# vovach777/llcomp

Measured on AMD Instinct MI355X. Metric: encode+decode MPix/s on 4K RGB8, bit-exact, higher is better.
Workload: dtype int32

## Files before the change

### llcomp_amd/csrc/dec_rows_asm.hpp

```cpp
#pragma once
#include <cstdint>

namespace llcomp_mi {

#define LD_E0L "v32"
#define LD_E0H "v33"
#define LD_E0 "v[32:33]"
#define LD_E5L "v34"
#define LD_E5H "v35"
#define LD_E5 "v[34:35]"
#define LD_E6L "v36"
#define LD_E6H "v37"
#define LD_E6 "v[36:37]"
#define LD_E7L "v38"
#define LD_E7H "v39"
#define LD_E7 "v[38:39]"
#define LD_E1L "v40"
#define LD_E1H "v41"
#define LD_E1 "v[40:41]"
#define LD_E2L "v42"
#define LD_E2H "v43"
#define LD_E2 "v[42:43]"
#define LD_E3L "v44"
#define LD_E3H "v45"
#define LD_E3 "v[44:45]"
#define LD_E4L "v48"
#define LD_E4H "v49"
#define LD_E4 "v[48:49]"
#define LD_PROD "v50"
#define LD_R1 "v51"
#define LD_DIFF "v52"
#define LD_OFF "v52"
#define LD_EX "v32"
#define LD_W "v33"
#define LD_RUN "v40"
#define LD_NX "v41"
#define LD_T "v42"
#define LD_SX "s[56:57]"
#define LD_SA "s[58:59]"
#define LD_SW "s[60:61]"
#define LD_SP "s[62:63]"
#define LD_S5 "s[64:65]"
#define LD_SB "s[64:65]"
#define LD_SU "s[66:67]"
#define LD_SD "s[68:69]"
#define LD_S1L "s[68:69]"
#define LD_SM "s[70:71]"
#define LD_S1 "s70"
#define LD_S2 "s71"

#define LD_SPLIT(EL)                                                                                                       \
    "v_mul_u32_u24_sdwa " LD_PROD ", " EL ", %[range] dst_sel:DWORD dst_unused:UNUSED_PAD src0_sel:BYTE_1 src1_sel:DWORD\n\t" \
    "v_lshrrev_b32_e32 " LD_R1 ", 8, " LD_PROD "\n\t"                                                                      \
    "v_sub_u32_e32 %[range], %[range], " LD_R1 "\n\t"
#define LD_SPLIT_IN(EL)                                                                                                       \
    "v_mul_u32_u24_sdwa " LD_PROD ", " EL ", %[range_in] dst_sel:DWORD dst_unused:UNUSED_PAD src0_sel:BYTE_1 src1_sel:DWORD\n\t" \
    "v_lshrrev_b32_e32 " LD_R1 ", 8, " LD_PROD "\n\t"                                                                      \
    "v_sub_u32_e32 %[range], %[range_in], " LD_R1 "\n\t"
#define LD_SPLIT_TO(EL, RD, WR)                                                                                       \
    "v_mul_u32_u24_sdwa " LD_PROD ", " EL ", " RD " dst_sel:DWORD dst_unused:UNUSED_PAD src0_sel:BYTE_1 src1_sel:DWORD\n\t" \
    "v_lshrrev_b32_e32 " WR ", 8, " LD_PROD "\n\t"                                                                     \
    "v_sub_u32_e32 " RD ", " RD ", " WR "\n\t"
#define LD_TAKE "v_lshlrev_b64 " LD_PAIR ", 8, " LD_PAIR "\n"
#define LD_REFILL(N)                                         \
    "v_cmp_gt_u32_e32 vcc, %[c100], %[range]\n\t"            \
    "s_and_saveexec_b64 " LD_SW ", vcc\n\t"                  \
    "s_cbranch_execz .Lrf" N "_%=\n\t"                       \
    "v_lshlrev_b32_e32 %[range], 8, %[range]\n\t"            \
    LD_TAKE                                                  \
    ".Lrf" N "_%=:\n\t"                                      \
    "s_mov_b64 exec, " LD_SW "\n\t"
#define LD_REFILL_R1(WR, N)                                       \
    "v_cmp_gt_u32_e32 vcc, %[c100], " WR "\n\t"                   \
    "s_and_saveexec_b64 " LD_SW ", vcc\n\t"                       \
    "s_cbranch_execz .Lrf" N "_%=\n\t"                            \
    "v_and_b32_e32 " WR ", 0xffffff00, " LD_PROD "\n\t"           \
    LD_TAKE                                                       \
    ".Lrf" N "_%=:\n\t"                                           \
    "s_mov_b64 exec, " LD_SW "\n\t"
#define LD_UNARY(EL, EH, OFS, N, SAVE, RD, WR)                              \
    LD_SPLIT_TO(EL, RD, WR)                                                 \
    "v_sub_co_u32_e32 " LD_LOW ", vcc, " LD_LOW ", " RD "\n\t"              \
    "ds_write_b16_d16_hi %[bank], " EL " offset:" OFS "\n\t"                \
    "s_andn2_b64 exec, exec, vcc\n\t"                                       \
    SAVE                                                                    \
    "s_cbranch_execz .Lx_done_%=\n\t"                                       \
    "ds_write_b16_d16_hi %[bank], " EH " offset:" OFS "\n\t"                \
    "v_add_u32_e32 " LD_EX ", 1, " LD_EX "\n\t"                             \
    LD_REFILL_R1(WR, N)
#define LD_FETCH_REST                                         \
    "v_lshrrev_b32_e32 " LD_E1L ", 16, %[w0]\n\t"             \
    "v_and_b32_e32 " LD_E2L ", 0xffff, %[w1]\n\t"             \
    "v_lshrrev_b32_e32 " LD_E3L ", 16, %[w1]\n\t"             \
    "v_and_b32_e32 " LD_E4L ", 0xffff, %[w2]\n\t"             \
    "ds_read_b64 " LD_E1 ", " LD_E1L "\n\t"                   \
    "ds_read_b64 " LD_E2 ", " LD_E2L "\n\t"                   \
    "ds_read_b64 " LD_E3 ", " LD_E3L "\n\t"                   \
    "ds_read_b64 " LD_E4 ", " LD_E4L "\n\t"                   \
    "v_lshrrev_b32_e32 " LD_E5L ", 16, %[w2]\n\t"             \
    "v_and_b32_e32 " LD_E6L ", 0xffff, %[w3]\n\t"             \
    "v_lshrrev_b32_e32 " LD_E7L ", 16, %[w3]\n\t"             \
    "ds_read_b64 " LD_E5 ", " LD_E5L "\n\t"                   \
    "ds_read_b64 " LD_E6 ", " LD_E6L "\n\t"                   \
    "ds_read_b64 " LD_E7 ", " LD_E7L "\n\t"

#define LD_HEAD_COPY "v_perm_b32 " LD_CPY ", %[winl_in], %[winl_in], %[sel]\n\t"
#define LD_SEL 0x0001020Du
#define LD_TAIL_BITS "v_ffbl_b32_e32 " LD_DIFF ", " LD_CPY "\n\t"
#define LD_URUN                                                      \
    ".Lu_%=:\n\t"                                                    \
    "s_waitcnt lgkmcnt(0)\n\t"                                       \
    LD_SPLIT_TO(LD_E4L, LD_R1, "%[range]")                           \
    "v_sub_co_u32_e32 " LD_LOW ", vcc, " LD_LOW ", " LD_R1 "\n\t"    \
    "s_and_b64 " LD_SP ", exec, vcc\n\t"                             \
    "s_andn2_b64 exec, exec, vcc\n\t"                                \
    "s_or_b64 " LD_SB ", " LD_SB ", " LD_SP "\n\t"                   \
    "s_cbranch_execz .Lu_done_%=\n\t"                                \
    "v_lshrrev_b32_e32 " LD_OFF ", 16, " LD_E4H "\n\t"               \
    "ds_read_b64 " LD_E4 ", " LD_OFF "\n\t"                          \
    "v_add_u32_e32 " LD_EX ", 1, " LD_EX "\n\t"                      \
    LD_REFILL_R1("%[range]", "4")                                    \
    "s_waitcnt lgkmcnt(0)\n\t"                                       \
    LD_SPLIT_TO(LD_E4L, "%[range]", LD_R1)                           \
    "v_sub_co_u32_e32 " LD_LOW ", vcc, " LD_LOW ", %[range]\n\t"     \
    "s_andn2_b64 exec, exec, vcc\n\t"                                \
    "s_cbranch_execz .Lu_done_%=\n\t"                                \
    "v_lshrrev_b32_e32 " LD_OFF ", 16, " LD_E4H "\n\t"               \
    "ds_read_b64 " LD_E4 ", " LD_OFF "\n\t"                          \
    "v_add_u32_e32 " LD_EX ", 1, " LD_EX "\n\t"                      \
    LD_REFILL_R1(LD_R1, "4b")                                        \
    "s_branch .Lu_%=\n"
#define LD_UNARY_INIT "s_mov_b64 " LD_SB ", 0\n\t"
#define LD_SAVE2 "s_mov_b64 " LD_SM ", exec\n\ts_andn2_b64 " LD_SB ", " LD_S1L ", exec\n\t"
#define LD_COLLECT                           \
    "s_mov_b64 exec, " LD_SB "\n\t"          \
    "v_mov_b32_e32 %[range], " LD_R1 "\n\t"

#define LD_TEXT                                                                                                                    \
        "s_mov_b64 " LD_SX ", exec\n\t"                                                                                            \
        LD_HEAD_COPY                                                                                                               \
        "v_and_b32_e32 " LD_OFF ", 0xffff, %[w0]\n\t"                                                                              \
        "ds_read_b64 " LD_E0 ", " LD_OFF "\n\t"                                                                                    \
        "v_mov_b32_e32 %[value], 0\n\t"                                                                                            \
        "s_cmp_lg_u32 %[hot], 0\n\t"                                                                                               \
        "s_cbranch_scc0 .Lcold_%=\n\t"                                                                                             \
        LD_FETCH_REST                                                                                                              \
        "s_waitcnt lgkmcnt(7)\n\t"                                                                                                 \
        "s_branch .Lzero_%=\n"                                                                                                     \
        ".Lcold_%=:\n\t"                                                                                                           \
        "s_waitcnt lgkmcnt(0)\n"                                                                                                   \
                                       \
        ".Lzero_%=:\n\t"                                                                                                           \
           \
                                          \
        LD_SPLIT_IN(LD_E0L)                                                                                                        \
        "v_sub_co_u32_e32 " LD_LOW ", vcc, %[low_in], %[range]\n\t"                                                                \
        "ds_write_b16_d16_hi %[bank], " LD_E0L "\n\t"                                                                              \
        "s_and_b64 " LD_SA ", exec, vcc\n\t"                                                                                       \
        "v_cndmask_b32_e32 " LD_LOW ", " LD_LOW ", %[low_in], vcc\n\t"                                                             \
        "s_andn2_b64 exec, exec, vcc\n\t"                                                                                          \
        "s_cbranch_execz .Lz1_%=\n\t"                                                                                              \
        "v_mov_b32_e32 %[range], " LD_R1 "\n\t"                                                                                    \
        "ds_write_b16_d16_hi %[bank], " LD_E0H "\n"                                                                                \
        ".Lz1_%=:\n\t"                                                                                                             \
        "s_mov_b64 exec, " LD_SX "\n\t"                                                                                            \
        LD_REFILL("0")                                                                                                             \
        "s_and_b64 exec, " LD_SA ", " LD_SA "\n\t"                                                                                 \
        "s_cbranch_execz .Ldone_%=\n\t"                                                                                            \
        "s_cmp_lg_u32 %[hot], 0\n\t"                                                                                               \
        "s_cbranch_scc1 .Lhave_%=\n\t"                                                                                             \
        LD_FETCH_REST                                                                                                              \
        ".Lhave_%=:\n\t"                                                                                                           \
        "v_mov_b32_e32 " LD_EX ", 0\n\t"                                                                                           \
        "v_mov_b32_e32 " LD_W ", 1\n\t"                                                                                            \
        "s_waitcnt lgkmcnt(0)\n\t"                                                                                                 \
                    \
           \
                                                       \
        "s_mov_b64 " LD_SM ", 0\n\t"                                                                                               \
        LD_UNARY_INIT                                                                                                              \
        LD_UNARY(LD_E1L, LD_E1H, "2", "1", "s_mov_b64 " LD_S1L ", exec\n\t", "%[range]", LD_R1)                                   \
        LD_UNARY(LD_E2L, LD_E2H, "256", "2", LD_SAVE2, LD_R1, "%[range]")                                                          \
        LD_UNARY(LD_E3L, LD_E3H, "258", "3", "", "%[range]", LD_R1)                                                                \
        "s_mov_b64 " LD_SU ", exec\n\t"                                                                                            \
        ".p2align 6\n"                                                                                                             \
        LD_URUN                                                                                                                    \
        ".Lu_done_%=:\n\t"                                                                                                         \
        "s_mov_b64 exec, " LD_SU "\n\t"                                                                                            \
        "ds_write_b16_d16_hi %[bank], " LD_E4L " offset:512\n"                             \
        ".Lx_done_%=:\n\t"                                                                                                         \
        LD_COLLECT                                                                                                                 \
        "s_mov_b64 exec, " LD_SA "\n\t"                                                                                            \
        "v_add_u32_e32 " LD_LOW ", " LD_LOW ", %[range]\n\t"     \
        LD_REFILL("5")                                                                   \
                                 \
        "v_cmp_lt_u32_e32 vcc, 31, " LD_EX "\n\t"                                                                                  \
        "s_cbranch_vccz .Lexok_%=\n\t"                                                                                             \
        "s_and_saveexec_b64 " LD_SP ", vcc\n\t"                                                                                    \
        "v_mov_b32_e32 " LD_CPY ", 0\n\t"        \
        "s_andn2_b64 exec, " LD_SP ", exec\n\t"                                                                                    \
        "s_cbranch_execz .Ldone_%=\n"                                                                                              \
        ".Lexok_%=:\n\t"                                                                                                           \
        "s_mov_b64 " LD_S5 ", exec\n\t"                             \
                                    \
        "s_and_b64 exec, exec, " LD_S1L "\n\t"                                                                  \
        "s_cbranch_execz .Lvalue_%=\n\t"                                                                                           \
        "s_mov_b64 " LD_SU ", exec\n\t"                                                                                            \
        LD_SPLIT(LD_E5L)                                                                                                           \
        "v_sub_co_u32_e32 " LD_DIFF ", vcc, " LD_LOW ", %[range]\n\t"                                                              \
        "ds_write_b16_d16_hi %[bank], " LD_E5L " offset:514\n\t"                                                                   \
        "s_andn2_b64 " LD_SP ", exec, vcc\n\t"                                                    \
        "v_addc_co_u32_e32 " LD_W ", vcc, " LD_W ", " LD_W ", vcc\n\t"                                        \
        "v_mov_b32_e32 " LD_RUN ", 0\n\t"                                                                                          \
        "s_and_b64 exec, " LD_SP ", " LD_SP "\n\t"                                                                                 \
        "s_cbranch_execz .Lp5_%=\n\t"                                                                                              \
        "v_mov_b32_e32 " LD_LOW ", " LD_DIFF "\n\t"                                                                                \
        "v_mov_b32_e32 %[range], " LD_R1 "\n\t"                                                                                    \
        "ds_write_b16_d16_hi %[bank], " LD_E5H " offset:514\n"                                                                     \
        ".Lp5_%=:\n\t"                                                                                                             \
        "s_mov_b64 exec, " LD_SU "\n\t"                                                                                            \
        LD_REFILL("6")                                                                                                             \
         \
        "v_add_u32_e32 " LD_T ", -1, " LD_EX "\n\t"                                                      \
        "s_and_b64 exec, exec, " LD_SM "\n\t"                                                                   \
        "s_cbranch_execz .Lm_skip_%=\n\t"                                                                                          \
        "s_mov_b64 " LD_SP ", exec\n\t"                                                                                            \
        "v_add_u32_e32 " LD_NX ", -2, " LD_EX "\n\t"                                                                               \
        "v_lshrrev_b32_e32 " LD_RUN ", " LD_NX ", %[sentv]\n\t"                                         \
        ".p2align 6\n"                                                                                                             \
        ".Lm_%=:\n\t"                                                                                                              \
        "s_waitcnt lgkmcnt(0)\n\t"                                                                                                 \
        LD_SPLIT(LD_E6L)                                                                                                           \
        "v_sub_co_u32_e32 " LD_DIFF ", vcc, " LD_LOW ", %[range]\n\t"                                                              \
        "s_nop 1\n\t"                                            \
        "v_cndmask_b32_e32 %[range], " LD_R1 ", %[range], vcc\n\t"                                                                 \
        "v_cndmask_b32_e32 " LD_LOW ", " LD_DIFF ", " LD_LOW ", vcc\n\t"                                                           \
        "v_cndmask_b32_e32 " LD_NX ", " LD_E6H ", " LD_E6L ", vcc\n\t"                                                             \
                                                            \
        "v_addc_co_u32_e32 " LD_RUN ", vcc, " LD_RUN ", " LD_RUN ", vcc\n\t"                                                       \
        "s_mov_b64 " LD_SD ", vcc\n\t"                                                                                             \
        "v_lshrrev_b32_e32 " LD_OFF ", 16, " LD_NX "\n\t"                                                                          \
        "ds_read_b64 " LD_E6 ", " LD_OFF "\n\t"                                                                                    \
        "v_cmp_gt_u32_e32 vcc, %[c100], %[range]\n\t"                                                                              \
        "s_and_saveexec_b64 " LD_SW ", vcc\n\t"                                                                                    \
        "s_cbranch_execz .Lmr_%=\n\t"                                                                                              \
        "v_lshlrev_b32_e32 %[range], 8, %[range]\n\t"                                                                              \
        LD_TAKE                                                                                                                    \
        ".Lmr_%=:\n\t"                                                                                                             \
        "s_andn2_b64 exec, " LD_SW ", " LD_SD "\n\t"                           \
        "s_cbranch_execnz .Lm_%=\n\t"                                                                                              \
        "s_mov_b64 exec, " LD_SP "\n\t"                                                                                            \
        "ds_write_b16_d16_hi %[bank], " LD_NX " offset:768\n"                       \
        ".Lm_skip_%=:\n\t"                                                                                                         \
        "s_mov_b64 exec, " LD_SU "\n\t"                                                                                            \
        "v_lshlrev_b32_e32 " LD_W ", " LD_T ", " LD_W "\n\t"   \
        "v_or_b32_e32 " LD_W ", " LD_W ", " LD_RUN "\n"                                                                            \
                                 \
        ".Lvalue_%=:\n\t"                                                                                                          \
        "s_mov_b64 exec, " LD_S5 "\n\t"                                                                                            \
        "v_lshlrev_b32_e64 " LD_T ", " LD_EX ", 1\n\t"                                                                             \
        "v_add_u32_e32 " LD_T ", -1, " LD_T "\n\t"                                                                                 \
        "v_xor_b32_e32 %[value], " LD_W ", " LD_T "\n\t"                                                                           \
                                                                                      \
        LD_SPLIT(LD_E7L)                                                                                                           \
        "v_sub_co_u32_e32 " LD_DIFF ", vcc, " LD_LOW ", %[range]\n\t"                                                              \
        "ds_write_b16_d16_hi %[bank], " LD_E7L " offset:770\n\t"                                                                   \
        "s_andn2_b64 exec, exec, vcc\n\t"                                                                                          \
        "s_cbranch_execz .Lp7_%=\n\t"                                                                                              \
        "v_mov_b32_e32 " LD_LOW ", " LD_DIFF "\n\t"                                                                                \
        "v_mov_b32_e32 %[range], " LD_R1 "\n\t"                                                                                    \
        "ds_write_b16_d16_hi %[bank], " LD_E7H " offset:770\n\t"                                                                   \
        "v_sub_u32_e32 %[value], 0, %[value]\n"                                                                                    \
        ".Lp7_%=:\n\t"                                                                                                             \
        "s_mov_b64 exec, " LD_S5 "\n\t"                                                                                            \
        LD_REFILL("7")                                                                                                             \
        ".Ldone_%=:\n\t"                                                                                                           \
        "s_mov_b64 exec, " LD_SX "\n\t"                                                                                            \
        LD_TAIL_BITS                                                                                                               \
        "v_lshrrev_b64 %[win], " LD_DIFF ", %[win_in]\n\t"              \
        "s_bcnt1_i32_b64 " LD_S1 ", " LD_SA "\n\t"                                                                                 \
        "s_bcnt1_i32_b64 " LD_S2 ", " LD_SX "\n\t"                                                                                 \
        "s_lshl_b32 " LD_S1 ", " LD_S1 ", 1\n\t"                                                                                   \
        "s_cmp_ge_u32 " LD_S1 ", " LD_S2 "\n\t"                                                                                    \
        "s_cselect_b32 %[hot], 1, 0\n\t"                                                                                           \
        "s_mov_b64 exec, " LD_SX "\n\t"
#define LD_INPUTS                                                                                                                   \
    [low_in] "v"(low_in), [range_in] "v"(range_in), [win_in] "v"(win_in), [winl_in] "v"(uint32_t(win_in)), [w0] "v"(w0), [w1] "v"(w1), \
        [w2] "v"(w2), [w3] "v"(w3), [bank] "v"(bank), [c100] "s"(0x100u), [sel] "s"(LD_SEL), [sentv] "v"(0x80000000u)
#define LD_CLOBBERS                                                                                                                 \
    "vcc", "scc", "memory", "v32", "v33", "v34", "v35", "v36", "v37", "v38", "v39", "v40", "v41", "v42", "v43", "v44", "v45", "v48", \
        "v49", "v50", "v51", "v52", "s56", "s57", "s58", "s59", "s60", "s61", "s62", "s63", "s64", "s65", "s66", "s67", "s68", "s69", \
        "s70", "s71"

#define LD_BLOCK(PAIR)                                                                                                        \
    asm volatile(LD_TEXT : [lc] "=&{" PAIR "}"(low_copy), [range] "=&v"(range), [win] "=&v"(win), [hot] "+s"(hot), [value] "=&v"(value) \
                 : LD_INPUTS                                                                                                  \
                 : LD_CLOBBERS)
#define LD_REPLAY_COPY(PAIR)                                                                  \
    asm("v_mov_b32_e32 " LD_LOW ", %3\n\tv_mov_b32_e32 %1, %4\n\tv_mov_b64_e32 %2, %5"        \
        : "+{" PAIR "}"(low_copy), "+v"(range), "+v"(win)                                     \
        : "v"(low_in), "v"(range_in), "v"(win_in))
template <int SET>
__device__ __forceinline__ void dec_rows_sample_asm(uint32_t low_in, uint32_t range_in, unsigned long long win_in,
                                                    unsigned long long& low_copy, uint32_t& range, unsigned long long& win, uint32_t w0,
                                                    uint32_t w1, uint32_t w2, uint32_t w3, uint32_t bank, uint32_t& hot, uint32_t& value) {
    if constexpr (SET == 0) {
#define LD_PAIR "v[0:1]"
#define LD_CPY "v0"
#define LD_LOW "v1"
        LD_BLOCK("v[0:1]");
    } else {
#undef LD_PAIR
#undef LD_CPY
#undef LD_LOW
#define LD_PAIR "v[2:3]"
#define LD_CPY "v2"
#define LD_LOW "v3"
        LD_BLOCK("v[2:3]");
    }
}
template <int SET>
__device__ __forceinline__ void dec_rows_replay_inputs(uint32_t low_in, uint32_t range_in, unsigned long long win_in,
                                                       unsigned long long& low_copy, uint32_t& range, unsigned long long& win) {
    if constexpr (SET == 0) {
#undef LD_LOW
#define LD_LOW "v1"
        LD_REPLAY_COPY("v[0:1]");
    } else {
#undef LD_LOW
#define LD_LOW "v3"
        LD_REPLAY_COPY("v[2:3]");
    }
}

}
```

### llcomp_amd/csrc/slice_kernels.hip

```cpp
#include <algorithm>
#include <type_traits>

#include "device_common.hpp"
#include "kernels.hpp"

#ifndef LLMI_ASM_ENC
#define LLMI_ASM_ENC 1
#endif
#if LLMI_ASM_ENC
#include "enc_rows_asm.hpp"
#endif
#ifndef LLMI_ASM_DEC
#define LLMI_ASM_DEC 1
#endif
#if LLMI_ASM_DEC
#include "dec_rows_asm.hpp"
#endif

namespace llcomp_mi {

namespace {

#ifdef LLMI_CLOCK_PROBE
constexpr uint32_t kProbeSlots = 1u << 15;
// ... 733 lines not shown
    }
}

template <int SLOT, bool INLDS>
__device__ __forceinline__ void dec_put_state(Bank& b, uint32_t half) {
    if constexpr (INLDS) *reinterpret_cast<uint16_t*>(b.lds + widebank_byte(SLOT)) = uint16_t(half >> 16);
    else set_slot_state<SLOT>(b.w, half & 0xFF);
}
template <int SLOT, bool INLDS>
__device__ __forceinline__ entry_t dec_entry(const Bank& b, const entry_t* tab) {
    if constexpr (INLDS) return lds_entry(wide_offset<SLOT>(b.w));
    else return tab[slot_state<SLOT>(b.w)];
}
template <bool INLDS>
__device__ __forceinline__ void dec_fetch_slot0(Entries& E, const Bank& b, const entry_t* tab) { E.e0 = dec_entry<0, INLDS>(b, tab); }
template <bool INLDS>
__device__ __forceinline__ void dec_fetch_rest(Entries& E, const Bank& b, const entry_t* tab) {
    E.e1 = dec_entry<1, INLDS>(b, tab);
    E.e2 = dec_entry<2, INLDS>(b, tab);
    E.e3 = dec_entry<3, INLDS>(b, tab);
    E.e4 = dec_entry<4, INLDS>(b, tab);
    E.e5 = dec_entry<5, INLDS>(b, tab);
    E.e6 = dec_entry<6, INLDS>(b, tab);
    E.e7 = dec_entry<7, INLDS>(b, tab);
}
struct RangeDec {
    uint32_t low, range;
    unsigned long long win;
    uint32_t nxt;
    const char* gbase;
    uint32_t ofs;
    uint32_t step;
    uint32_t ofs_end;
    uint32_t replays;
};
__device__ __forceinline__ bool window_low(const RangeDec& d) { return uint32_t(d.win >> 32) == 0; }
__device__ __forceinline__ void dec_prefetch(RangeDec& d) {
    d.nxt = *reinterpret_cast<const uint32_t*>(d.gbase + min(d.ofs, d.ofs_end));
    d.ofs += d.step;
}
__device__ __forceinline__ uint32_t consume_here(uint32_t v) {
    asm volatile("" : "+v"(v) : : "memory");
    return v;
}
__device__ __forceinline__ void dec_append(RangeDec& d) {
    const uint32_t ready = consume_here(d.nxt);
    const uint32_t sh = 31u - uint32_t(__builtin_clz(uint32_t(d.win)));
    const uint32_t rest = uint32_t(d.win) ^ (1u << sh);
    d.win = ((0x100000000ull | ready) << sh) | rest;
    dec_prefetch(d);
}
__device__ __forceinline__ void dec_append_drained(RangeDec& d) {
    dec_append(d);
    drain_vector_memory();
}
__device__ __forceinline__ void dec_open(RangeDec& d, const uint32_t* group, uint32_t lane, uint32_t shift, uint32_t len) {
    d.gbase = reinterpret_cast<const char*>(group);
    d.ofs = lane * 4;
    d.step = 4u << shift;
    asm volatile("" : "+v"(d.step));
    d.ofs_end = lane * 4 + ((len + 3) >> 2) * d.step;
    dec_prefetch(d);
    const uint32_t first = d.nxt;
    dec_prefetch(d);
    const unsigned long long both = first | ((unsigned long long)d.nxt << 32);
    dec_prefetch(d);
    d.range = 0xFF00;
    d.low = ((first & 0xFF) << 8) | ((first >> 8) & 0xFF);
    d.win = (both >> 16) | (1ull << 48);
    d.replays = 0;
}
__device__ __forceinline__ unsigned long long window_next(unsigned long long w) {
    unsigned long long r;
    asm("v_lshrrev_b64 %0, 8, %1" : "=v"(r) : "v"(w));
    return r;
}
__device__ __forceinline__ void dec_refill(RangeDec& d) {
    if (d.range < 0x100) {
        d.range <<= 8;
        d.low = (d.low << 8) | (uint32_t(d.win) & 0xFF);
        d.win = window_next(d.win);
    }
}
template <bool CHECKED>
__device__ __forceinline__ bool dec_core(RangeDec& d, uint32_t P) {
    if (CHECKED && d.win <= 1) dec_append_drained(d);
    const uint32_t r1 = __umul24(d.range, P) >> 8;
    const uint32_t r0 = d.range - r1;
    uint32_t diff;
    const bool under = __builtin_usub_overflow(d.low, r0, &diff);
    const bool bit = !under;
    d.low = under ? d.low : diff;
    d.range = under ? r0 : r1;
    dec_refill(d);
    return bit;
}
template <bool CHECKED>
__device__ __forceinline__ uint32_t dec_step_acc(RangeDec& d, uint32_t P, entry_t cur, uint32_t& w) {
    if (CHECKED && d.win <= 1) dec_append_drained(d);
    const uint32_t r1 = __umul24(d.range, P) >> 8;
    const uint32_t r0 = d.range - r1;
    uint32_t diff, nx;
    asm("v_sub_co_u32_e32 %[diff], vcc, %[low], %[r0]\n\t"
        "s_nop 1\n\t"
        "v_cndmask_b32_e32 %[range], %[r1], %[r0], vcc\n\t"
        "v_cndmask_b32_e32 %[low], %[diff], %[low], vcc\n\t"
        "v_cndmask_b32_e32 %[nx], %[hi], %[lo], vcc\n\t"
        "v_addc_co_u32_e32 %[w], vcc, %[w], %[w], vcc"
        : [diff] "=&v"(diff), [range] "=&v"(d.range), [low] "+v"(d.low), [nx] "=&v"(nx), [w] "+v"(w)
        : [r0] "v"(r0), [r1] "v"(r1), [lo] "v"(uint32_t(cur)), [hi] "v"(uint32_t(cur >> 32))
        : "vcc");
    if (d.range < 0x100) {
        d.range <<= 8;
        d.low = (d.low << 8) | (uint32_t(d.win) & 0xFF);
        d.win = window_next(d.win);
    }
    return nx;
}
template <int SLOT, bool CHECKED, bool INLDS>
__device__ __forceinline__ bool dec_once(RangeDec& d, Bank& bank, const Entries& E) {
    const entry_t en = E.get<SLOT>();
    const bool bit = dec_core<CHECKED>(d, prob_of(en));
    dec_put_state<SLOT, INLDS>(bank, successor(en, bit));
    return bit;
}
template <bool ALL, bool CHECKED, bool INLDS>
__device__ __forceinline__ bool dec_residual(RangeDec& d, Bank& bank, const entry_t* tab, uint32_t& out) {
    Entries E;
    dec_fetch_slot0<INLDS>(E, bank, tab);
    if (ALL) dec_fetch_rest<INLDS>(E, bank, tab);
    if (dec_once<0, CHECKED, INLDS>(d, bank, E)) {
        out = 0;
        return true;
    }
    if (!ALL) dec_fetch_rest<INLDS>(E, bank, tab);
    int ex = 0;
    bool ok = true;
    if (dec_once<1, CHECKED, INLDS>(d, bank, E)) {
        ex = 1;
        if (dec_once<2, CHECKED, INLDS>(d, bank, E)) {
            ex = 2;
            if (dec_once<3, CHECKED, INLDS>(d, bank, E)) {
                entry_t cur = E.e4;
                int n = 0;
                for (;;) {
                    if (CHECKED && d.win <= 1) dec_append_drained(d);
                    const uint32_t r1 = __umul24(d.range, prob_of(cur)) >> 8;
                    d.range -= r1;
                    ++n;
                    asm volatile("" : "+v"(n));
                    uint32_t diff;
                    if (__builtin_usub_overflow(d.low, d.range, &diff)) break;
                    d.low = diff;
                    d.range = r1;
                    if (CHECKED && n > 29) break;
                    cur = entry_at(tab, uint32_t(cur >> 32));
                    dec_refill(d);
                }
                dec_refill(d);
                ex = 2 + n;
                if (ex > 31) ok = false;
                const uint32_t nx = uint32_t(cur);
                dec_put_state<4, INLDS>(bank, nx);
            }
        }
    }
    if (!ok) return false;
    uint32_t w = 1;
    const uint32_t ones = (1u << ex) - 1;
    if (ex > 0) {
        w += w + uint32_t(!dec_once<5, CHECKED, INLDS>(d, bank, E));
        if (ex > 1) {
            entry_t cur = E.e6;
            uint32_t nx;
            uint32_t limit = ones + 1;
            asm volatile("" : "+v"(limit));
            do {
                nx = dec_step_acc<CHECKED>(d, prob_of(cur), cur, w);
                cur = entry_at(tab, nx);
            } while (w < limit);
            dec_put_state<6, INLDS>(bank, nx);
        }
    }
    uint32_t v = w ^ ones;
    if (dec_once<7, CHECKED, INLDS>(d, bank, E)) v = 0u - v;
    out = v;
    return true;
}

template <bool INLDS, int SET = 0>
__device__ __forceinline__ bool dec_sample(RangeDec& d, Bank& bank, const entry_t* tab, uint32_t& hot, bool replay_always,
                                           uint32_t& v) {
#if LLMI_ASM_DEC
    if constexpr (INLDS) {
        uint32_t range;
        unsigned long long low_left, win;
        dec_rows_sample_asm<SET>(d.low, d.range, d.win, low_left, range, win, bank.w[0], bank.w[1], bank.w[2], bank.w[3], lds_address(bank.lds),
                                 hot, v);
        if (__builtin_expect(uint32_t(low_left) == 0 || replay_always, 0)) {
            ++d.replays;
            reinterpret_cast<uint32_t*>(bank.lds)[0] = bank.w[0];
            reinterpret_cast<uint32_t*>(bank.lds)[64] = bank.w[1];
            reinterpret_cast<uint32_t*>(bank.lds)[128] = bank.w[2];
            reinterpret_cast<uint32_t*>(bank.lds)[192] = bank.w[3];
            dec_rows_replay_inputs<SET>(d.low, d.range, d.win, low_left, range, win);
            d.low = uint32_t(low_left >> 32);
            d.range = range;
            d.win = win;
            return dec_residual<false, true, true>(d, bank, tab, v);
        }
        d.low = uint32_t(low_left >> 32);
        d.range = range;
        d.win = win;
        return true;
    } else
#endif
    {
        const uint32_t s_low = d.low, s_range = d.range, s_b0 = bank.w[0], s_b1 = bank.w[1], s_b2 = bank.w[2], s_b3 = bank.w[3];
        const unsigned long long s_win = d.win;
        bool ok = hot ? dec_residual<true, false, INLDS>(d, bank, tab, v) : dec_residual<false, false, INLDS>(d, bank, tab, v);
        hot = 2 * __popcll(__ballot(v != 0)) >= __popcll(__ballot(true));
        if (__builtin_expect(!ok || d.win == 0 || replay_always, 0)) {
            ++d.replays;
            d.low = s_low; d.range = s_range; d.win = s_win;
            bank.w[0] = s_b0; bank.w[1] = s_b1;
            if constexpr (INLDS) {
                bank.w[2] = s_b2; bank.w[3] = s_b3;
                reinterpret_cast<uint32_t*>(bank.lds)[0] = s_b0;
                reinterpret_cast<uint32_t*>(bank.lds)[64] = s_b1;
                reinterpret_cast<uint32_t*>(bank.lds)[128] = s_b2;
                reinterpret_cast<uint32_t*>(bank.lds)[192] = s_b3;
            }
            ok = dec_residual<false, true, INLDS>(d, bank, tab, v);
        }
        return ok;
    }
}

constexpr uint32_t bank_cache_lds_bytes(int log2_entries) { return log2_entries ? (64u * 9u) << log2_entries : 0u; }
template <int NCH, bool ROWS, bool LDSTAB = false, int CACHE = 0, bool SMALL = false>
__global__ __launch_bounds__(64, ROWS && NCH == 1 ? 8 : 1) void k_decode_slices(const Geometry g, const uint32_t lpw_and_flags,
                                                      const uint8_t* __restrict__ units,
                                                      const uint32_t* __restrict__ slice_len,
                                                      uint64_t* __restrict__ states, int16_t* __restrict__ rec,
                                                      uint32_t* status, const uint64_t gpat,
                                                      unsigned long long* __restrict__ counters) {
    __shared__ entry_t tab[128];
    __shared__ uint32_t rowbank[ROWS ? kWideBankWords : 1];
    __shared__ int8_t quant_lut[ROWS ? 1 : 512];
    if constexpr (!ROWS) {
        for (uint32_t i = threadIdx.x; i < 256; i += blockDim.x) {
            quant_lut[i] = int8_t(quant11(int(i) - 128));
            quant_lut[256 + i] = int8_t(quant5(int(i) - 128));
        }
    }
    static_assert(CACHE == 0 || (!ROWS && !LDSTAB && NCH != 0), "the bank cache belongs to the 2-D kernels with tables in HBM");
    static_assert(!SMALL || ROWS, "the model is a template flag of the 1-row-slice kernels only");
    static_assert(CACHE == 0 || ((kContexts - 1) >> CACHE) < 0xFF, "bank cache: a context's tag would alias the empty marker");
    __shared__ uint32_t wave_sums[CACHE != 0 ? 2 : 1];
    clear_lds_states<LDSTAB>();
    if constexpr (CACHE != 0) {
        uint32_t* tg = reinterpret_cast<uint32_t*>(dyn_lds + (512u << CACHE));
        for (uint32_t i = threadIdx.x; i < (16u << CACHE); i += blockDim.x) tg[i] = 0xFFFFFFFFu;
        if (threadIdx.x < 2) wave_sums[threadIdx.x] = 0;
    }
    load_table(tab);
    const uint32_t lpw = lpw_and_flags & 0xFF;
    const bool replay_always = (lpw_and_flags >> 8) & 1;
    [[maybe_unused]] const bool small_model = (g.flags & kGeoSmallModel) != 0;
    const uint32_t id = blockIdx.x * lpw + threadIdx.x;
    if (threadIdx.x >= lpw || id >= g.n_slices) return;
    const SliceRect r = slice_rect(g, id);
    RangeDec d;
    const uint32_t len = min(slice_len[id], g.slice_cap - 16);
    const uint32_t grp = __builtin_amdgcn_readfirstlane(id >> g.lane_shift);
    const uint32_t lane_in_group = id & ((1u << g.lane_shift) - 1);
    dec_open(d, reinterpret_cast<const uint32_t*>(units) + ((size_t(grp) * (g.slice_cap >> 2)) << g.lane_shift), lane_in_group,
             g.lane_shift, len);

    int16_t* p0 = rec + lane_order_index(g, id, 0);
    const ptrdiff_t GW = ptrdiff_t(1) << g.lane_shift;
    int16_t* const gbase = rec + ((size_t(grp) * g.slice_samples) << g.lane_shift);
    uint32_t hot = 0;
    LLMI_PROBE_START();

    if constexpr (ROWS) {
        for (uint32_t k = 0; k < 12; ++k) rowbank[k * 64 + threadIdx.x] = lds_address(tab) * 0x00010001u;
        int l[NCH], L[NCH];
#pragma unroll
        for (int k = 0; k < NCH; ++k) l[k] = L[k] = 128;
        int held_val = 0;
        uint32_t store_ofs = lane_in_group * 2, step_ofs = 2u << g.lane_shift;
        asm volatile("" : "+v"(step_ofs));
        uint8_t* const bank0 = reinterpret_cast<uint8_t*>(rowbank) + threadIdx.x * 4;
        bool bad = false;
        auto pixel = [&](auto model, auto start, auto set) {
            constexpr int MODEL = decltype(model)::value;
            constexpr bool START = decltype(start)::value;
            constexpr int SET = decltype(set)::value;
#pragma unroll
            for (int k = 0; k < NCH; ++k) {
                if (window_low(d)) dec_append(d);
                if (!(START && k == 0)) {
                    asm volatile("global_store_short %0, %1, %2" : : "v"(store_ofs), "v"(held_val), "s"(gbase) : "memory");
                    store_ofs += step_ofs;
                }
                const int lv = l[k];
                uint32_t sg = 0, bofs = 0;
                if constexpr (MODEL != kModelSmall) {
                    const int dq = L[k] - lv;
                    sg = uint32_t(dq >> 31);
                    asm volatile("" : "+v"(sg));
                    const uint32_t aq = (uint32_t(dq) ^ sg) - sg;
                    uint32_t o1 = ((aq + 0x7FFFFFFFu) >> 21) & 0x400u, o2 = ((aq + 0x7FFFFFFCu) >> 21) & 0x400u;
                    asm volatile("" : "+v"(o1), "+v"(o2));
                    bofs = o1 + o2;
                }
                uint32_t* bp = reinterpret_cast<uint32_t*>(bank0 + bofs);
                Bank bank{{bp[0], bp[64], bp[128], bp[192]}, reinterpret_cast<uint8_t*>(bp)};
                uint32_t v = 0;
                const bool ok = ((SET + k) & 1) ? dec_sample<true, 1>(d, bank, tab, hot, replay_always, v)
                                                : dec_sample<true, 0>(d, bank, tab, hot, replay_always, v);
                if (!ok) bad = true;
                if constexpr (MODEL != kModelSmall) v = (v ^ sg) - sg;
                const int val = int(int16_t(uint32_t(lv) + v));
                held_val = val;
                L[k] = START ? val : lv;
                l[k] = val;
            }
        };
        const uint32_t sw0 = __builtin_amdgcn_readfirstlane(r.sw);
        const uint32_t n_bulk = __builtin_amdgcn_ballot_w64(r.sw != sw0) == 0 ? sw0 : 0;
        uint32_t x = 1;
        constexpr std::integral_constant<int, 0> set0{};
        constexpr std::integral_constant<int, 1> set1{};
        pixel(no_model, std::true_type{}, set0);
        constexpr std::integral_constant<int, SMALL ? kModelSmall : kModelLarge> model{};
        if constexpr (NCH == 1) {
            for (; x + 1 < n_bulk; x += 2) {
                pixel(model, std::false_type{}, set1);
                pixel(model, std::false_type{}, set0);
            }
        } else {
            for (; x < n_bulk; ++x) pixel(model, std::false_type{}, set0);
        }
        for (; x < r.sw; ++x) pixel(model, std::false_type{}, set1);
        if (bad) atomicOr(status, kStBadExponent);
        asm volatile("global_store_short %0, %1, %2" : : "v"(store_ofs), "v"(held_val), "s"(gbase) : "memory");
        publish_count(counters, kCtrDecReplays, d.replays);
    } else {
        uint64_t* banks;
        uint32_t bsh;
        if constexpr (LDSTAB) {
            banks = reinterpret_cast<uint64_t*>(dyn_lds);
            bsh = 0;
        } else {
            banks = states + ((size_t(id >> g.lane_shift) * kContexts) << g.lane_shift) + (id & ((1u << g.lane_shift) - 1));
            bsh = g.lane_shift;
        }
        if constexpr (NCH == 0) {
            const uint32_t nch = g.nch;
            const ptrdiff_t px_step = ptrdiff_t(nch) * GW, up = ptrdiff_t(r.sw) * px_step;
            for (uint32_t y = 0; y < r.sh; ++y) {
                for (uint32_t x = 0; x < r.sw; ++x) {
                    for (uint32_t k = 0; k < nch; ++k) {
                        int16_t* q = p0 + ptrdiff_t(y) * up + ptrdiff_t(x) * px_step + ptrdiff_t(k) * GW;
                        if (window_low(d)) dec_append(d);
                        const Hood n = apply_borders(x > 0 ? q[-px_step] : 0, x > 1 ? q[-2 * px_step] : 0, y > 0 ? q[-up] : 0,
                                                     (y > 0 && x > 0) ? q[-up - px_step] : 0, (y > 0 && x + 1 < r.sw) ? q[-up + px_step] : 0,
                                                     y > 1 ? q[-2 * up] : 0, x, y, r.sw);
                        int ctx = context_hash(n, small_model);
                        const bool neg = ctx < 0;
                        if (neg) ctx = -ctx;
                        const uint64_t b64 = bank_fresh<LDSTAB>(banks[size_t(ctx) << bsh], gpat);
                        Bank bank{{uint32_t(b64), uint32_t(b64 >> 32)}, nullptr};
                        uint32_t v;
                        if (!dec_sample<false>(d, bank, tab, hot, replay_always, v)) {
                            atomicOr(status, kStBadExponent);
                            return;
                        }
                                banks[size_t(ctx) << bsh] = bank_tagged<LDSTAB>(uint64_t(bank.w[0]) | (uint64_t(bank.w[1]) << 32), gpat);
                        if (neg) v = 0u - v;
                        *q = int16_t(uint32_t(predict(n)) + v);
                    }
                }
            }
            publish_count(counters, kCtrDecReplays, d.replays);
        } else {
        const ptrdiff_t up = ptrdiff_t(r.sw) * NCH * GW;
        uint32_t held_ctx = ~0u;
        uint64_t held_bank = 0;
        [[maybe_unused]] uint64_t wb_bank = 0;
        [[maybe_unused]] uint64_t* wb_ptr = nullptr;
        [[maybe_unused]] bool use_cache = CACHE != 0;
        [[maybe_unused]] uint32_t my_miss = 0, my_lookups = 0, my_wb = 0, miss_mark = 0, look_mark = 0;
        LLMI_PARTS_DECL();
        LLMI_PARTS_START();
        for (uint32_t y = 0; y < r.sh; ++y) {
            if constexpr (CACHE != 0) {
                const uint32_t yu = __builtin_amdgcn_readfirstlane(y);
                if (use_cache && yu >= 4 && (yu & 3) == 0) {
                    __hip_atomic_fetch_add(&wave_sums[0], my_miss - miss_mark, __ATOMIC_RELAXED, __HIP_MEMORY_SCOPE_WORKGROUP);
                    __hip_atomic_fetch_add(&wave_sums[1], my_lookups - look_mark, __ATOMIC_RELAXED, __HIP_MEMORY_SCOPE_WORKGROUP);
                    miss_mark = my_miss;
                    look_mark = my_lookups;
// ... 267 lines not shown
```

Measured before the change: 31080.

## Track low-minus-range offset state in asm row decoder to shorten bit decisions

Changes the range decoder's internal state from `low` to `low - range` (a signed offset), so each binary decision is a single add with carry instead of subtract, compare and conditional move. The split, unary-run and sign steps in the inline asm are rewritten around that, and the value is now accumulated directly into the output register instead of being XOR-fixed at the end. This removes several VALU ops and a cndmask per decoded bit on the hot path. It adds state conversions at entry and exit and at the replay fallback, and it forces replay for lanes whose low is at least range.

Measured after the change: 31010, median of 2. About the same (-0.2%).

```diff
diff --git a/llcomp_amd/csrc/dec_rows_asm.hpp b/llcomp_amd/csrc/dec_rows_asm.hpp
--- a/llcomp_amd/csrc/dec_rows_asm.hpp
+++ b/llcomp_amd/csrc/dec_rows_asm.hpp
@@ -30,9 +30,10 @@
 #define LD_PROD "v50"
 #define LD_R1 "v51"
 #define LD_DIFF "v52"
+#define LD_SUM "v52"
 #define LD_OFF "v52"
 #define LD_EX "v32"
-#define LD_W "v33"
+#define LD_W "%[value]"
 #define LD_RUN "v40"
 #define LD_NX "v41"
 #define LD_T "v42"
@@ -59,8 +60,7 @@
     "v_sub_u32_e32 %[range], %[range_in], " LD_R1 "\n\t"
 #define LD_SPLIT_TO(EL, RD, WR)                                                                                       \
     "v_mul_u32_u24_sdwa " LD_PROD ", " EL ", " RD " dst_sel:DWORD dst_unused:UNUSED_PAD src0_sel:BYTE_1 src1_sel:DWORD\n\t" \
-    "v_lshrrev_b32_e32 " WR ", 8, " LD_PROD "\n\t"                                                                     \
-    "v_sub_u32_e32 " RD ", " RD ", " WR "\n\t"
+    "v_lshrrev_b32_e32 " WR ", 8, " LD_PROD "\n\t"
 #define LD_TAKE "v_lshlrev_b64 " LD_PAIR ", 8, " LD_PAIR "\n"
 #define LD_REFILL(N)                                         \
     "v_cmp_gt_u32_e32 vcc, %[c100], %[range]\n\t"            \
@@ -80,9 +80,9 @@
     "s_mov_b64 exec, " LD_SW "\n\t"
 #define LD_UNARY(EL, EH, OFS, N, SAVE, RD, WR)                              \
     LD_SPLIT_TO(EL, RD, WR)                                                 \
-    "v_sub_co_u32_e32 " LD_LOW ", vcc, " LD_LOW ", " RD "\n\t"              \
+    "v_add_co_u32_e32 " LD_SUM ", vcc, " LD_LOW ", " WR "\n\t"              \
     "ds_write_b16_d16_hi %[bank], " EL " offset:" OFS "\n\t"                \
-    "s_andn2_b64 exec, exec, vcc\n\t"                                       \
+    "s_and_b64 exec, exec, vcc\n\t"                                         \
     SAVE                                                                    \
     "s_cbranch_execz .Lx_done_%=\n\t"                                       \
     "ds_write_b16_d16_hi %[bank], " EH " offset:" OFS "\n\t"                \
@@ -111,9 +111,9 @@
     ".Lu_%=:\n\t"                                                    \
     "s_waitcnt lgkmcnt(0)\n\t"                                       \
     LD_SPLIT_TO(LD_E4L, LD_R1, "%[range]")                           \
-    "v_sub_co_u32_e32 " LD_LOW ", vcc, " LD_LOW ", " LD_R1 "\n\t"    \
-    "s_and_b64 " LD_SP ", exec, vcc\n\t"                             \
-    "s_andn2_b64 exec, exec, vcc\n\t"                                \
+    "v_add_co_u32_e32 " LD_SUM ", vcc, " LD_LOW ", %[range]\n\t"     \
+    "s_andn2_b64 " LD_SP ", exec, vcc\n\t"                           \
+    "s_and_b64 exec, exec, vcc\n\t"                                  \
     "s_or_b64 " LD_SB ", " LD_SB ", " LD_SP "\n\t"                   \
     "s_cbranch_execz .Lu_done_%=\n\t"                                \
     "v_lshrrev_b32_e32 " LD_OFF ", 16, " LD_E4H "\n\t"               \
@@ -122,8 +122,8 @@
     LD_REFILL_R1("%[range]", "4")                                    \
     "s_waitcnt lgkmcnt(0)\n\t"                                       \
     LD_SPLIT_TO(LD_E4L, "%[range]", LD_R1)                           \
-    "v_sub_co_u32_e32 " LD_LOW ", vcc, " LD_LOW ", %[range]\n\t"     \
-    "s_andn2_b64 exec, exec, vcc\n\t"                                \
+    "v_add_co_u32_e32 " LD_SUM ", vcc, " LD_LOW ", " LD_R1 "\n\t"    \
+    "s_and_b64 exec, exec, vcc\n\t"                                  \
     "s_cbranch_execz .Lu_done_%=\n\t"                                \
     "v_lshrrev_b32_e32 " LD_OFF ", 16, " LD_E4H "\n\t"               \
     "ds_read_b64 " LD_E4 ", " LD_OFF "\n\t"                          \
@@ -132,9 +132,13 @@
     "s_branch .Lu_%=\n"
 #define LD_UNARY_INIT "s_mov_b64 " LD_SB ", 0\n\t"
 #define LD_SAVE2 "s_mov_b64 " LD_SM ", exec\n\ts_andn2_b64 " LD_SB ", " LD_S1L ", exec\n\t"
-#define LD_COLLECT                           \
-    "s_mov_b64 exec, " LD_SB "\n\t"          \
-    "v_mov_b32_e32 %[range], " LD_R1 "\n\t"
+#define LD_COLLECT                                               \
+    "s_mov_b64 exec, " LD_SB "\n\t"                              \
+    "v_sub_u32_e32 %[range], " LD_R1 ", %[range]\n\t"            \
+    "s_andn2_b64 exec, " LD_SA ", " LD_SB "\n\t"                 \
+    "v_sub_u32_e32 %[range], %[range], " LD_R1 "\n\t"            \
+    "s_mov_b64 exec, " LD_SA "\n\t"                              \
+    "v_mov_b32_e32 " LD_LOW ", " LD_SUM "\n\t"
 
 #define LD_TEXT                                                                                                                    \
         "s_mov_b64 " LD_SX ", exec\n\t"                                                                                            \
@@ -149,18 +153,18 @@
         "s_branch .Lzero_%=\n"                                                                                                     \
         ".Lcold_%=:\n\t"                                                                                                           \
         "s_waitcnt lgkmcnt(0)\n"                                                                                                   \
-                                       \
+                                        \
         ".Lzero_%=:\n\t"                                                                                                           \
-           \
-                                          \
+         \
+                                                         \
         LD_SPLIT_IN(LD_E0L)                                                                                                        \
-        "v_sub_co_u32_e32 " LD_LOW ", vcc, %[low_in], %[range]\n\t"                                                                \
+        "v_add_co_u32_e32 " LD_LOW ", vcc, %[d_in], " LD_R1 "\n\t"                                                               \
         "ds_write_b16_d16_hi %[bank], " LD_E0L "\n\t"                                                                              \
-        "s_and_b64 " LD_SA ", exec, vcc\n\t"                                                                                       \
-        "v_cndmask_b32_e32 " LD_LOW ", " LD_LOW ", %[low_in], vcc\n\t"                                                             \
-        "s_andn2_b64 exec, exec, vcc\n\t"                                                                                          \
+        "s_andn2_b64 " LD_SA ", exec, vcc\n\t"                                                                                     \
+        "s_and_b64 exec, exec, vcc\n\t"                                                                                            \
         "s_cbranch_execz .Lz1_%=\n\t"                                                                                              \
         "v_mov_b32_e32 %[range], " LD_R1 "\n\t"                                                                                    \
+        "v_mov_b32_e32 " LD_LOW ", %[d_in]\n\t"                                                                                  \
         "ds_write_b16_d16_hi %[bank], " LD_E0H "\n"                                                                                \
         ".Lz1_%=:\n\t"                                                                                                             \
         "s_mov_b64 exec, " LD_SX "\n\t"                                                                                            \
@@ -176,7 +180,7 @@
         "s_waitcnt lgkmcnt(0)\n\t"                                                                                                 \
                     \
            \
-                                                       \
+                                           \
         "s_mov_b64 " LD_SM ", 0\n\t"                                                                                               \
         LD_UNARY_INIT                                                                                                              \
         LD_UNARY(LD_E1L, LD_E1H, "2", "1", "s_mov_b64 " LD_S1L ", exec\n\t", "%[range]", LD_R1)                                   \
@@ -189,32 +193,32 @@
         "s_mov_b64 exec, " LD_SU "\n\t"                                                                                            \
         "ds_write_b16_d16_hi %[bank], " LD_E4L " offset:512\n"                             \
         ".Lx_done_%=:\n\t"                                                                                                         \
-        LD_COLLECT                                                                                                                 \
-        "s_mov_b64 exec, " LD_SA "\n\t"                                                                                            \
-        "v_add_u32_e32 " LD_LOW ", " LD_LOW ", %[range]\n\t"     \
-        LD_REFILL("5")                                                                   \
+        LD_COLLECT      \
+        LD_REFILL("5")                                                               \
                                  \
         "v_cmp_lt_u32_e32 vcc, 31, " LD_EX "\n\t"                                                                                  \
         "s_cbranch_vccz .Lexok_%=\n\t"                                                                                             \
         "s_and_saveexec_b64 " LD_SP ", vcc\n\t"                                                                                    \
         "v_mov_b32_e32 " LD_CPY ", 0\n\t"        \
+        "v_mov_b32_e32 %[value], 0\n\t"                           \
         "s_andn2_b64 exec, " LD_SP ", exec\n\t"                                                                                    \
         "s_cbranch_execz .Ldone_%=\n"                                                                                              \
         ".Lexok_%=:\n\t"                                                                                                           \
         "s_mov_b64 " LD_S5 ", exec\n\t"                             \
-                                    \
+         \
+                                                        \
         "s_and_b64 exec, exec, " LD_S1L "\n\t"                                                                  \
-        "s_cbranch_execz .Lvalue_%=\n\t"                                                                                           \
+        "s_cbranch_execz .Lsign_%=\n\t"                                                                                            \
         "s_mov_b64 " LD_SU ", exec\n\t"                                                                                            \
         LD_SPLIT(LD_E5L)                                                                                                           \
-        "v_sub_co_u32_e32 " LD_DIFF ", vcc, " LD_LOW ", %[range]\n\t"                                                              \
+        "v_add_co_u32_e32 " LD_LOW ", vcc, " LD_LOW ", " LD_R1 "\n\t"                                                              \
         "ds_write_b16_d16_hi %[bank], " LD_E5L " offset:514\n\t"                                                                   \
-        "s_andn2_b64 " LD_SP ", exec, vcc\n\t"                                                    \
-        "v_addc_co_u32_e32 " LD_W ", vcc, " LD_W ", " LD_W ", vcc\n\t"                                        \
+        "s_and_b64 " LD_SP ", exec, vcc\n\t"                                                      \
+        "v_addc_co_u32_e32 " LD_W ", vcc, " LD_W ", " LD_W ", vcc\n\t"                                         \
         "v_mov_b32_e32 " LD_RUN ", 0\n\t"                                                                                          \
         "s_and_b64 exec, " LD_SP ", " LD_SP "\n\t"                                                                                 \
         "s_cbranch_execz .Lp5_%=\n\t"                                                                                              \
-        "v_mov_b32_e32 " LD_LOW ", " LD_DIFF "\n\t"                                                                                \
+        "v_sub_u32_e32 " LD_LOW ", " LD_LOW ", " LD_R1 "\n\t"                                                                      \
         "v_mov_b32_e32 %[range], " LD_R1 "\n\t"                                                                                    \
         "ds_write_b16_d16_hi %[bank], " LD_E5H " offset:514\n"                                                                     \
         ".Lp5_%=:\n\t"                                                                                                             \
@@ -231,12 +235,12 @@
         ".Lm_%=:\n\t"                                                                                                              \
         "s_waitcnt lgkmcnt(0)\n\t"                                                                                                 \
         LD_SPLIT(LD_E6L)                                                                                                           \
-        "v_sub_co_u32_e32 " LD_DIFF ", vcc, " LD_LOW ", %[range]\n\t"                                                              \
+        "v_add_co_u32_e32 " LD_DIFF ", vcc, " LD_LOW ", " LD_R1 "\n\t"                                                             \
         "s_nop 1\n\t"                                            \
-        "v_cndmask_b32_e32 %[range], " LD_R1 ", %[range], vcc\n\t"                                                                 \
+        "v_cndmask_b32_e32 %[range], %[range], " LD_R1 ", vcc\n\t"        \
         "v_cndmask_b32_e32 " LD_LOW ", " LD_DIFF ", " LD_LOW ", vcc\n\t"                                                           \
-        "v_cndmask_b32_e32 " LD_NX ", " LD_E6H ", " LD_E6L ", vcc\n\t"                                                             \
-                                                            \
+        "v_cndmask_b32_e32 " LD_NX ", " LD_E6L ", " LD_E6H ", vcc\n\t"                                                             \
+                                                                   \
         "v_addc_co_u32_e32 " LD_RUN ", vcc, " LD_RUN ", " LD_RUN ", vcc\n\t"                                                       \
         "s_mov_b64 " LD_SD ", vcc\n\t"                                                                                             \
         "v_lshrrev_b32_e32 " LD_OFF ", 16, " LD_NX "\n\t"                                                                          \
@@ -255,19 +259,15 @@
         "s_mov_b64 exec, " LD_SU "\n\t"                                                                                            \
         "v_lshlrev_b32_e32 " LD_W ", " LD_T ", " LD_W "\n\t"   \
         "v_or_b32_e32 " LD_W ", " LD_W ", " LD_RUN "\n"                                                                            \
-                                 \
-        ".Lvalue_%=:\n\t"                                                                                                          \
+                  \
+        ".Lsign_%=:\n\t"                                                                                                           \
         "s_mov_b64 exec, " LD_S5 "\n\t"                                                                                            \
-        "v_lshlrev_b32_e64 " LD_T ", " LD_EX ", 1\n\t"                                                                             \
-        "v_add_u32_e32 " LD_T ", -1, " LD_T "\n\t"                                                                                 \
-        "v_xor_b32_e32 %[value], " LD_W ", " LD_T "\n\t"                                                                           \
-                                                                                      \
         LD_SPLIT(LD_E7L)                                                                                                           \
-        "v_sub_co_u32_e32 " LD_DIFF ", vcc, " LD_LOW ", %[range]\n\t"                                                              \
+        "v_add_co_u32_e32 " LD_LOW ", vcc, " LD_LOW ", " LD_R1 "\n\t"                                                              \
         "ds_write_b16_d16_hi %[bank], " LD_E7L " offset:770\n\t"                                                                   \
-        "s_andn2_b64 exec, exec, vcc\n\t"                                                                                          \
+        "s_and_b64 exec, exec, vcc\n\t"                                                                                            \
         "s_cbranch_execz .Lp7_%=\n\t"                                                                                              \
-        "v_mov_b32_e32 " LD_LOW ", " LD_DIFF "\n\t"                                                                                \
+        "v_sub_u32_e32 " LD_LOW ", " LD_LOW ", " LD_R1 "\n\t"                                                                      \
         "v_mov_b32_e32 %[range], " LD_R1 "\n\t"                                                                                    \
         "ds_write_b16_d16_hi %[bank], " LD_E7H " offset:770\n\t"                                                                   \
         "v_sub_u32_e32 %[value], 0, %[value]\n"                                                                                    \
@@ -285,7 +285,7 @@
         "s_cselect_b32 %[hot], 1, 0\n\t"                                                                                           \
         "s_mov_b64 exec, " LD_SX "\n\t"
 #define LD_INPUTS                                                                                                                   \
-    [low_in] "v"(low_in), [range_in] "v"(range_in), [win_in] "v"(win_in), [winl_in] "v"(uint32_t(win_in)), [w0] "v"(w0), [w1] "v"(w1), \
+    [d_in] "v"(d_in), [range_in] "v"(range_in), [win_in] "v"(win_in), [winl_in] "v"(uint32_t(win_in)), [w0] "v"(w0), [w1] "v"(w1), \
         [w2] "v"(w2), [w3] "v"(w3), [bank] "v"(bank), [c100] "s"(0x100u), [sel] "s"(LD_SEL), [sentv] "v"(0x80000000u)
 #define LD_CLOBBERS                                                                                                                 \
     "vcc", "scc", "memory", "v32", "v33", "v34", "v35", "v36", "v37", "v38", "v39", "v40", "v41", "v42", "v43", "v44", "v45", "v48", \
@@ -293,16 +293,16 @@
         "s70", "s71"
 
 #define LD_BLOCK(PAIR)                                                                                                        \
-    asm volatile(LD_TEXT : [lc] "=&{" PAIR "}"(low_copy), [range] "=&v"(range), [win] "=&v"(win), [hot] "+s"(hot), [value] "=&v"(value) \
+    asm volatile(LD_TEXT : [lc] "=&{" PAIR "}"(d_copy), [range] "=&v"(range), [win] "=&v"(win), [hot] "+s"(hot), [value] "=&v"(value) \
                  : LD_INPUTS                                                                                                  \
                  : LD_CLOBBERS)
-#define LD_REPLAY_COPY(PAIR)                                                                  \
-    asm("v_mov_b32_e32 " LD_LOW ", %3\n\tv_mov_b32_e32 %1, %4\n\tv_mov_b64_e32 %2, %5"        \
-        : "+{" PAIR "}"(low_copy), "+v"(range), "+v"(win)                                     \
-        : "v"(low_in), "v"(range_in), "v"(win_in))
+#define LD_REPLAY_COPY(PAIR)                                                                     \
+    asm("v_add_u32_e32 " LD_LOW ", %3, %4\n\tv_mov_b32_e32 %1, %4\n\tv_mov_b64_e32 %2, %5"        \
+        : "+{" PAIR "}"(low_copy), "+v"(range), "+v"(win)                                        \
+        : "v"(d_in), "v"(range_in), "v"(win_in))
 template <int SET>
-__device__ __forceinline__ void dec_rows_sample_asm(uint32_t low_in, uint32_t range_in, unsigned long long win_in,
-                                                    unsigned long long& low_copy, uint32_t& range, unsigned long long& win, uint32_t w0,
+__device__ __forceinline__ void dec_rows_sample_asm(uint32_t d_in, uint32_t range_in, unsigned long long win_in,
+                                                    unsigned long long& d_copy, uint32_t& range, unsigned long long& win, uint32_t w0,
                                                     uint32_t w1, uint32_t w2, uint32_t w3, uint32_t bank, uint32_t& hot, uint32_t& value) {
     if constexpr (SET == 0) {
 #define LD_PAIR "v[0:1]"
@@ -320,7 +320,7 @@
     }
 }
 template <int SET>
-__device__ __forceinline__ void dec_rows_replay_inputs(uint32_t low_in, uint32_t range_in, unsigned long long win_in,
+__device__ __forceinline__ void dec_rows_replay_inputs(uint32_t d_in, uint32_t range_in, unsigned long long win_in,
                                                        unsigned long long& low_copy, uint32_t& range, unsigned long long& win) {
     if constexpr (SET == 0) {
 #undef LD_LOW
diff --git a/llcomp_amd/csrc/slice_kernels.hip b/llcomp_amd/csrc/slice_kernels.hip
--- a/llcomp_amd/csrc/slice_kernels.hip
+++ b/llcomp_amd/csrc/slice_kernels.hip
@@ -839,25 +839,41 @@
         d.win = window_next(d.win);
     }
 }
-template <bool CHECKED>
+template <bool SGN>
+__device__ __forceinline__ bool dec_under(uint32_t low, uint32_t r0, uint32_t& diff) {
+    if constexpr (SGN) {
+        diff = low - r0;
+        return int32_t(low) < int32_t(r0);
+    } else {
+        return __builtin_usub_overflow(low, r0, &diff);
+    }
+}
+template <bool CHECKED, bool SGN = false>
 __device__ __forceinline__ bool dec_core(RangeDec& d, uint32_t P) {
     if (CHECKED && d.win <= 1) dec_append_drained(d);
     const uint32_t r1 = __umul24(d.range, P) >> 8;
     const uint32_t r0 = d.range - r1;
     uint32_t diff;
-    const bool under = __builtin_usub_overflow(d.low, r0, &diff);
+    const bool under = dec_under<SGN>(d.low, r0, diff);
     const bool bit = !under;
     d.low = under ? d.low : diff;
     d.range = under ? r0 : r1;
     dec_refill(d);
     return bit;
 }
-template <bool CHECKED>
+template <bool CHECKED, bool SGN = false>
 __device__ __forceinline__ uint32_t dec_step_acc(RangeDec& d, uint32_t P, entry_t cur, uint32_t& w) {
     if (CHECKED && d.win <= 1) dec_append_drained(d);
     const uint32_t r1 = __umul24(d.range, P) >> 8;
     const uint32_t r0 = d.range - r1;
     uint32_t diff, nx;
+    if constexpr (SGN) {
+        const bool under = dec_under<true>(d.low, r0, diff);
+        d.range = under ? r0 : r1;
+        d.low = under ? d.low : diff;
+        nx = under ? uint32_t(cur) : uint32_t(cur >> 32);
+        w += w + uint32_t(under);
+    } else
     asm("v_sub_co_u32_e32 %[diff], vcc, %[low], %[r0]\n\t"
         "s_nop 1\n\t"
         "v_cndmask_b32_e32 %[range], %[r1], %[r0], vcc\n\t"
@@ -877,7 +893,7 @@
 template <int SLOT, bool CHECKED, bool INLDS>
 __device__ __forceinline__ bool dec_once(RangeDec& d, Bank& bank, const Entries& E) {
     const entry_t en = E.get<SLOT>();
-    const bool bit = dec_core<CHECKED>(d, prob_of(en));
+    const bool bit = dec_core<CHECKED, CHECKED && INLDS>(d, prob_of(en));
     dec_put_state<SLOT, INLDS>(bank, successor(en, bit));
     return bit;
 }
@@ -907,7 +923,7 @@
                     ++n;
                     asm volatile("" : "+v"(n));
                     uint32_t diff;
-                    if (__builtin_usub_overflow(d.low, d.range, &diff)) break;
+                    if (dec_under<CHECKED && INLDS>(d.low, d.range, diff)) break;
                     d.low = diff;
                     d.range = r1;
                     if (CHECKED && n > 29) break;
@@ -933,7 +949,7 @@
             uint32_t limit = ones + 1;
             asm volatile("" : "+v"(limit));
             do {
-                nx = dec_step_acc<CHECKED>(d, prob_of(cur), cur, w);
+                nx = dec_step_acc<CHECKED, CHECKED && INLDS>(d, prob_of(cur), cur, w);
                 cur = entry_at(tab, nx);
             } while (w < limit);
             dec_put_state<6, INLDS>(bank, nx);
@@ -964,7 +980,9 @@
             d.low = uint32_t(low_left >> 32);
             d.range = range;
             d.win = win;
-            return dec_residual<false, true, true>(d, bank, tab, v);
+            const bool ok = dec_residual<false, true, true>(d, bank, tab, v);
+            d.low -= d.range;
+            return ok;
         }
         d.low = uint32_t(low_left >> 32);
         d.range = range;
@@ -1051,6 +1069,10 @@
         asm volatile("" : "+v"(step_ofs));
         uint8_t* const bank0 = reinterpret_cast<uint8_t*>(rowbank) + threadIdx.x * 4;
         bool bad = false;
+        const bool replay_lane = replay_always || d.low >= d.range;
+#if LLMI_ASM_DEC
+        d.low -= d.range;
+#endif
         auto pixel = [&](auto model, auto start, auto set) {
             constexpr int MODEL = decltype(model)::value;
             constexpr bool START = decltype(start)::value;
@@ -1076,8 +1098,8 @@
                 uint32_t* bp = reinterpret_cast<uint32_t*>(bank0 + bofs);
                 Bank bank{{bp[0], bp[64], bp[128], bp[192]}, reinterpret_cast<uint8_t*>(bp)};
                 uint32_t v = 0;
-                const bool ok = ((SET + k) & 1) ? dec_sample<true, 1>(d, bank, tab, hot, replay_always, v)
-                                                : dec_sample<true, 0>(d, bank, tab, hot, replay_always, v);
+                const bool ok = ((SET + k) & 1) ? dec_sample<true, 1>(d, bank, tab, hot, replay_lane, v)
+                                                : dec_sample<true, 0>(d, bank, tab, hot, replay_lane, v);
                 if (!ok) bad = true;
                 if constexpr (MODEL != kModelSmall) v = (v ^ sg) - sg;
                 const int val = int(int16_t(uint32_t(lv) + v));
```
